# raulmur/ORB_SLAM2

Hardware: NVIDIA H100
Metric: stereo frames/sec (ORB extract L+R + ComputeStereoMatches, KITTI-shaped 1242x375 @2000 kpts) (higher is better)
Workload: dtype u8

## Files before the change

### orb_slam2_b200/csrc/borb_host.cu

```cuda
#include <cmath>
#include <cstdarg>
#include <cstdio>
#include <algorithm>
#include <cstdlib>
#include <cstring>

#include "borb_internal.h"

namespace borb {

static thread_local std::string tl_error;
void set_error(const char* fmt, ...) {
    char buf[512];
    va_list ap;
    va_start(ap, fmt);
    vsnprintf(buf, sizeof(buf), fmt, ap);
    va_end(ap);
    tl_error = buf;
}

bool allow_max_smem(const void* func) {
    static std::mutex mu;
    static std::vector<std::pair<const void*, int>> done;
    int dev = 0;
    if (cudaGetDevice(&dev) != cudaSuccess) return false;
    std::lock_guard<std::mutex> lk(mu);
    for (auto& d : done)
        if (d.first == func && d.second == dev) return true;
    cudaFuncAttributes fa;
    int optin = 0;
    cudaError_t e = cudaFuncGetAttributes(&fa, func);
    if (e == cudaSuccess) e = cudaDeviceGetAttribute(&optin, cudaDevAttrMaxSharedMemoryPerBlockOptin, dev);
    if (e == cudaSuccess) e = cudaFuncSetAttribute(func, cudaFuncAttributeMaxDynamicSharedMemorySize, optin - (int)fa.sharedSizeBytes);
    if (e != cudaSuccess) { set_error("raising the shared-memory limit failed: %s", cudaGetErrorString(e)); cudaGetLastError(); return false; }
    done.push_back({func, dev});
    return true;
}

namespace {

inline int cv_round_f(float v) { return (int)lrintf(v); }
inline int align_up(int v, int a) { return (v + a - 1) / a * a; }

void init_tables(borb_extractor* e) {
    const int L = e->cfg.n_levels;
    const double sf = (double)e->cfg.scale_factor;
    e->scale.assign(L, 1.f); e->sigma2.assign(L, 1.f); e->inv_scale.assign(L, 1.f); e->inv_sigma2.assign(L, 1.f);
    for (int i = 1; i < L; i++) {
        e->scale[i] = (float)((double)e->scale[i - 1] * sf);
        e->sigma2[i] = e->scale[i] * e->scale[i];
    }
    for (int i = 0; i < L; i++) { e->inv_scale[i] = 1.0f / e->scale[i]; e->inv_sigma2[i] = 1.0f / e->sigma2[i]; }
    e->per_level.assign(L, 0);
    const float factor = (float)(1.0 / sf);
    float want = (float)e->cfg.n_features * (1.f - factor) / (1.f - (float)std::pow((double)factor, (double)L));
    int sum = 0;
    for (int l = 0; l < L - 1; l++) {
        e->per_level[l] = cv_round_f(want);
        sum += e->per_level[l];
        want *= factor;
    }
    e->per_level[L - 1] = e->cfg.n_features - sum > 0 ? e->cfg.n_features - sum : 0;
    const int vmax = (int)std::floor(HALF_PATCH * std::sqrt(2.f) / 2 + 1);
    const int vmin = (int)std::ceil(HALF_PATCH * std::sqrt(2.f) / 2);
    for (int v = 0; v < 16; v++) e->umax[v] = 0;
    for (int v = 0; v <= vmax; ++v) e->umax[v] = (int)lrint(std::sqrt((double)HALF_PATCH * HALF_PATCH - (double)v * v));
    for (int v = HALF_PATCH, v0 = 0; v >= vmin; --v) {
        while (e->umax[v0] == e->umax[v0 + 1]) ++v0;
        e->umax[v] = v0;
        ++v0;
    }
}

void resize_table(int src, int dst, bool clamp_edges, int extra, std::vector<int16_t>& out) {
    const double inv = (double)dst / src, scale = 1. / inv;
    const size_t first = out.size();
    for (int d = 0; d < dst; d++) {
        float f = (float)((d + 0.5) * scale - 0.5);
        int s = (int)std::floor(f);
        f -= s;
        if (clamp_edges) {
            if (s < 0) { f = 0; s = 0; }
            if (s >= src - 1) { f = 0; s = src - 1; }
        }
        out.push_back((int16_t)s);
        out.push_back((int16_t)cv_round_f((1.f - f) * 2048.f));
        out.push_back((int16_t)cv_round_f(f * 2048.f));
        out.push_back(0);
    }
    for (int k = 0; k < extra; k++) {
        int r = 2 * dst - 2 - (dst + k);
        if (r < 0) r = 0;
        for (int j = 0; j < 4; j++) out.push_back(out[first + (size_t)r * 4 + j]);
    }
    if (((out.size() - first) / 4) & 1) for (int j = 0; j < 4; j++) out.push_back(0);
}

bool resize_window_table(const std::vector<int16_t>& tabs, size_t xtab_first, int n_entries, std::vector<int16_t>& out) {
    bool ok = true;
    for (int gq = 0; gq < n_entries; gq += 4) {
        int lo = 1 << 30, hi = 0;
        for (int i = 0; i < 4; i++) {
            const int ofs = tabs[xtab_first + (size_t)(gq + i) * 4];
            lo = std::min(lo, ofs); hi = std::max(hi, ofs);
        }
        const int base = lo & ~3;
        if (hi + 1 - base > 11) ok = false;
        for (int i = 0; i < 4; i++) {
            const int16_t* e = &tabs[xtab_first + (size_t)(gq + i) * 4];
            const int pos = e[0] - base;
            int s1 = 0, s2 = 0x10;
            if (pos <= 6) s1 = pos | ((pos + 1) << 4);
            else if (pos == 7) { s1 = 7; s2 = 0x40; }
            else { const int q = (pos - 8) + 4; s2 = q | ((q + 1) << 4); }
            out.push_back(e[1]);
            out.push_back(e[2]);
            out.push_back((int16_t)base);
            out.push_back((int16_t)((s1 | (s2 << 8)) & 0x7FFF));
        }
    }
    return ok;
}

const int8_t kPattern[1024] = {
#include "orb_pattern.inc"
};

borb_status build_geometry(borb_extractor* e, int w, int h, std::vector<int16_t>& tabs) {
    Geometry& g = e->geom;
    std::memset(&g, 0, sizeof(g));
    const int L = e->cfg.n_levels;
    g.nlevels = L; g.w = w; g.h = h;
    g.fast_mode = e->fast_mode;
    g.ini_th = e->cfg.ini_th_fast < 0 ? 0 : (e->cfg.ini_th_fast > 255 ? 255 : e->cfg.ini_th_fast);
    g.min_th = e->cfg.min_th_fast < 0 ? 0 : (e->cfg.min_th_fast > 255 ? 255 : e->cfg.min_th_fast);
    for (int i = 0; i < 16; i++) g.umax[i] = e->umax[i];
    unsigned pyr_off = 0, cand_off = 0;
    int blk = 0, sel_off = 0, btile = 0;
    tabs.clear();
    for (int l = 0; l < L; l++) {
        LevelGeom& v = g.lv[l];
        v.w = cv_round_f((float)w * e->inv_scale[l]);
        v.h = cv_round_f((float)h * e->inv_scale[l]);
        const float width = (float)(v.w - 2 * MIN_BORDER), height = (float)(v.h - 2 * MIN_BORDER);
        v.nCols = (int)(width / 30.f);
        v.nRows = (int)(height / 30.f);
        if (v.nCols < 1 || v.nRows < 1) {
            set_error("level %d is %dx%d: too small for the 30-px FAST cell grid (reference divides by zero)", l, v.w, v.h);
            return BORB_ERR_UNSUPPORTED;
        }
        v.wCell = (int)std::ceil(width / v.nCols);
        v.hCell = (int)std::ceil(height / v.nRows);
        v.pitch = align_up(v.w + 8, 128);
        v.pyr_off = pyr_off;
        pyr_off += (unsigned)v.pitch * v.h;
        v.cellsPerBlk = FAST_TILE_W / v.wCell > 0 ? FAST_TILE_W / v.wCell : 1;
        v.blkCols = (v.nCols + v.cellsPerBlk - 1) / v.cellsPerBlk;
        v.blkBase = blk;
        blk += v.blkCols * v.nRows;
        v.cand_off = cand_off;
        v.cand_cap = v.nCols * v.nRows * ((v.wCell + 1) / 2) * ((v.hCell + 1) / 2);
        cand_off += (unsigned)align_up(v.cand_cap, 32);
        v.quota = e->per_level[l];
        v.nIni = (int)std::round(width / height);
        if (v.nIni < 1) { set_error("level %d aspect ratio gives zero quadtree roots (reference divides by zero)", l); return BORB_ERR_UNSUPPORTED; }
        v.hX = width / v.nIni;
        v.node_cap = (v.quota > 4 * v.nIni ? v.quota : 4 * v.nIni) + 3;
        v.node_cap = align_up(v.node_cap + 1, 4);
        v.sel_off = sel_off;
        sel_off += v.node_cap;
        v.scale = e->scale[l];
        v.inv_scale = e->inv_scale[l];
        v.patch_size = (float)(int)(PATCH * e->scale[l]);
        g.blur_base[l] = btile;
        btile += ((v.w + BLUR_TILE_W - 1) / BLUR_TILE_W) * ((v.h + BLUR_TILE_H - 1) / BLUR_TILE_H);
        if (l > 0) {
            const int wpad = (v.w + 8 + 3) & ~3;
            v.xtab_off = (unsigned)(tabs.size() / 4);
            resize_table(g.lv[l - 1].w, v.w, true, wpad - v.w, tabs);
            v.ytab_off = (unsigned)(tabs.size() / 4);
            resize_table(g.lv[l - 1].h, v.h, false, 0, tabs);
            v.xwin_off = (unsigned)(tabs.size() / 4);
            std::vector<int16_t> win;
            v.x_windowed = resize_window_table(tabs, (size_t)v.xtab_off * 4, wpad, win) ? 1 : 0;
            tabs.insert(tabs.end(), win.begin(), win.end());
        }
        if (quadtree_smem_bytes(v.node_cap) > 200 * 1024) {
            set_error("per-level quota %d exceeds the quadtree kernel's shared-memory envelope", v.quota);
            return BORB_ERR_UNSUPPORTED;
        }
    }
    g.blur_base[L] = btile;
    g.blur_tiles = btile;
    g.fast_blocks = blk;
    g.pyr_image_stride = (unsigned)align_up((int)pyr_off, g.lv[0].pitch);
    g.cand_image_stride = cand_off;
    g.sel_image_stride = sel_off;
    if (sel_off >= 65536) { set_error("keypoint capacity %d exceeds 65535", sel_off); return BORB_ERR_UNSUPPORTED; }
    return BORB_OK;
}

void free_workspace(Workspace& ws) {
    cudaFree(ws.pyr); cudaFree(ws.blur); cudaFree(ws.cand); cudaFree(ws.cand_cnt); cudaFree(ws.pnode); cudaFree(ws.sel);
    cudaFree(ws.sel_cnt); cudaFree(ws.kps); cudaFree(ws.desc); cudaFree(ws.nkp); cudaFree(ws.u_right); cudaFree(ws.depth);
    cudaFree(ws.sad); cudaFree(ws.tabs); cudaFree(ws.brief_slots); cudaFree(ws.pair_idx); cudaFree(ws.st_bins); cudaFree(ws.st_recs); cudaFree(ws.stage);
    free(ws.fast_tmaps); cudaFree(ws.fast_tiles);
    ws = Workspace();
}

borb_status ensure(borb_extractor* e, int w, int h, int n_images) {
    if (w < 1 || h < 1 || w > BORB_MAX_DIM || h > BORB_MAX_DIM) { set_error("image size %dx%d outside [1,%d]", w, h, BORB_MAX_DIM); return BORB_ERR_UNSUPPORTED; }
    BORB_CUDA(cudaSetDevice(e->device));
    const bool same_shape = e->have_geom && e->geom.w == w && e->geom.h == h;
    if (same_shape && e->ws.max_images >= n_images) return BORB_OK;
    BORB_CUDA(cudaStreamSynchronize(e->stream));
    std::vector<int16_t> tabs;
    e->have_geom = false;
    e->last_n_images = 0;
    e->last_stereo_pairs = 0;
    borb_status st = build_geometry(e, w, h, tabs);
    if (st != BORB_OK) return st;
    size_t n = (size_t)(n_images > 2 ? n_images : 2);
    if (same_shape && (size_t)e->ws.max_images > n) n = (size_t)e->ws.max_images;
    free_workspace(e->ws);
    if (e->h_counts) { cudaFreeHost(e->h_counts); e->h_counts = nullptr; }
    e->pair_cache.clear();
    const Geometry& g = e->geom;
    Workspace& ws = e->ws;
    BORB_CUDA(cudaMalloc(&ws.pyr, n * g.pyr_image_stride + 256));
    BORB_CUDA(cudaMalloc(&ws.blur, n * g.pyr_image_stride + 256));
    BORB_CUDA(cudaMalloc(&ws.cand, n * g.cand_image_stride * sizeof(uint32_t)));
    BORB_CUDA(cudaMalloc(&ws.pnode, n * g.cand_image_stride * sizeof(int)));
    BORB_CUDA(cudaMalloc(&ws.cand_cnt, n * g.nlevels * sizeof(int)));
    BORB_CUDA(cudaMalloc(&ws.sel, n * g.sel_image_stride * sizeof(uint32_t)));
    BORB_CUDA(cudaMalloc(&ws.sel_cnt, n * g.nlevels * sizeof(int)));
    BORB_CUDA(cudaMalloc(&ws.kps, n * g.sel_image_stride * sizeof(borb_keypoint)));
    BORB_CUDA(cudaMalloc(&ws.desc, n * g.sel_image_stride * 32));
    BORB_CUDA(cudaMalloc(&ws.nkp, n * sizeof(int)));
    BORB_CUDA(cudaMalloc(&ws.u_right, n * g.sel_image_stride * sizeof(float)));
    BORB_CUDA(cudaMalloc(&ws.depth, n * g.sel_image_stride * sizeof(float)));
    BORB_CUDA(cudaMalloc(&ws.sad, n * g.sel_image_stride * sizeof(int)));
    BORB_CUDA(cudaMalloc(&ws.pair_idx, n * 2 * sizeof(int)));
    BORB_CUDA(cudaMalloc(&ws.st_bins, n * stereo_bins_bytes_per_pair()));
    BORB_CUDA(cudaMalloc(&ws.st_recs, n * (size_t)stereo_rec_stride(g) * stereo_rec_bytes()));
    BORB_CUDA(cudaMalloc(&ws.tabs, (tabs.size() + 4) * sizeof(int16_t)));
    BORB_CUDA(cudaMemcpy(ws.tabs, tabs.data(), tabs.size() * sizeof(int16_t), cudaMemcpyHostToDevice));
    const std::vector<uint32_t>& slots = brief_slot_table();
    BORB_CUDA(cudaMalloc(&ws.brief_slots, slots.size() * sizeof(uint32_t)));
    BORB_CUDA(cudaMemcpy(ws.brief_slots, slots.data(), slots.size() * sizeof(uint32_t), cudaMemcpyHostToDevice));
    BORB_CUDA(cudaMemset(ws.nkp, 0, n * sizeof(int)));
    BORB_CUDA(cudaMallocHost(&e->h_counts, n * 2 * sizeof(int)));
    ws.max_images = (int)n;
    ws.fast_tmaps = malloc(fast_tmaps_bytes());
    if ((st = build_fast_tmaps(g, ws, ws.fast_tmaps)) != BORB_OK) return st;
    if ((st = build_fast_tiles(g, ws)) != BORB_OK) return st;
    e->have_geom = true;
    return BORB_OK;
}

void drain_timing(borb_extractor* e);
void begin_step(borb_extractor* e) {
    if (!e->timing) return;
    if (e->ev.empty()) {
        e->ev.resize((size_t)borb_extractor::EV_RING * 9);
        for (auto& x : e->ev) cudaEventCreate(&x);
    }
    if (e->ev_pending >= borb_extractor::EV_RING) {
        cudaStreamSynchronize(e->stream);
        drain_timing(e);
    }
    e->ev_slot = (e->ev_slot + 1) % borb_extractor::EV_RING;
    e->ev_mask[e->ev_slot] = 0;
    e->ev_pending++;
}
void mark(borb_extractor* e, int i) {
    if (!e->timing || e->ev.empty()) return;
    cudaEventRecord(e->ev[(size_t)e->ev_slot * 9 + i], e->stream);
    e->ev_mask[e->ev_slot] |= 1u << i;
}
void drain_timing(borb_extractor* e) {
    const int R = borb_extractor::EV_RING;
    for (int k = e->ev_pending - 1; k >= 0; k--) {
        const int slot = ((e->ev_slot - k) % R + R) % R;
        const unsigned m = e->ev_mask[slot];
        for (int i = 0; i < 8; i++) {
            float ms = 0.f;
            if (m & (1u << i)) {
                int j = i + 1;
                while (j < 9 && !(m & (1u << j))) j++;
                if (j < 9 && cudaEventElapsedTime(&ms, e->ev[(size_t)slot * 9 + i], e->ev[(size_t)slot * 9 + j]) != cudaSuccess) { ms = 0.f; cudaGetLastError(); }
            }
            e->stage_ms[i] = ms;
            e->stage_sum_ms[i] += ms;
        }
        e->stage_steps++;
    }
    e->ev_pending = 0;
}

borb_status enqueue_extract(borb_extractor* e, int n) {
    const Geometry& g = e->geom;
    Workspace& ws = e->ws;
    cudaStream_t s = e->stream;
    BORB_CUDA(cudaMemsetAsync(ws.cand_cnt, 0, (size_t)n * g.nlevels * sizeof(int), s));
    mark(e, 1);
    e->launches += launch_pyramid(g, ws, n, s);
    mark(e, 2);
    e->launches += launch_fast(g, ws, n, s);
    mark(e, 3);
    e->launches += launch_quadtree(g, ws, n, s);
    mark(e, 4);
    e->launches += launch_blur(g, ws, n, s);
    mark(e, 5);
    e->launches += launch_describe(g, ws, n, s);
    mark(e, 6);
    BORB_CUDA(cudaGetLastError());
    e->last_n_images = n;
    e->last_stereo_pairs = 0;
    return BORB_OK;
}

borb_status rectified_size(borb_extractor* e, int w, int h, int* gw, int* gh) {
    if (!e->d_map[0][0]) return BORB_OK;
    if (w != e->map_src_w || h != e->map_src_h) {
        set_error("rectification maps were built for %dx%d raw frames, got %dx%d", e->map_src_w, e->map_src_h, w, h);
        return BORB_ERR_INVALID_ARG;
    }
    *gw = e->map_dst_w; *gh = e->map_dst_h;
    return BORB_OK;
}

borb_status upload_slots(borb_extractor* e, const uint8_t* const* slots, int n, int w, int h, int stride, bool stereo_pairs = false) {
    const Geometry& g = e->geom;
    const int ch = e->in_channels;
    if (stride < w * ch) { set_error("stride %d smaller than a row of %d %d-channel pixels", stride, w, ch); return BORB_ERR_INVALID_ARG; }
    const size_t img_bytes = (size_t)stride * h;
    bool contiguous = n > 1 || ch > 1 || e->d_map[0][0] != nullptr;
    for (int k = 0; k < n; k++) {
        if (!slots[k]) { set_error("image %d is NULL", k); return BORB_ERR_INVALID_ARG; }
        if (slots[k] != slots[0] + (size_t)k * img_bytes) contiguous = false;
    }
    auto need_stage = [&](size_t need) -> borb_status {
        if (e->ws.stage_bytes < need) {
            BORB_CUDA(cudaStreamSynchronize(e->stream));
            cudaFree(e->ws.stage);
            e->ws.stage = nullptr; e->ws.stage_bytes = 0;
            BORB_CUDA(cudaMalloc(&e->ws.stage, need));
            e->ws.stage_bytes = need;
        }
        return BORB_OK;
    };
    if (e->d_map[0][0]) {
        if (ch != 1) { set_error("rectification maps apply to CV_8UC1 frames"); return BORB_ERR_UNSUPPORTED; }
        const size_t src_img = contiguous ? img_bytes : (size_t)w * h;
        const int src_stride = contiguous ? stride : w;
        borb_status st = need_stage(src_img * n);
        if (st != BORB_OK) return st;
        if (contiguous) BORB_CUDA(cudaMemcpyAsync(e->ws.stage, slots[0], src_img * n, cudaMemcpyHostToDevice, e->stream));
        else
            for (int k = 0; k < n; k++)
                BORB_CUDA(cudaMemcpy2DAsync(e->ws.stage + (size_t)k * src_img, w, slots[k], stride, w, h, cudaMemcpyHostToDevice, e->stream));
        e->launches += launch_repack_remap(g, e->ws, e->ws.stage, src_stride, src_img, w, h, e->d_map[0][0], e->d_map[0][1],
                                           stereo_pairs ? e->d_map[1][0] : nullptr, stereo_pairs ? e->d_map[1][1] : nullptr, n, e->stream);
        return BORB_OK;
    }
    if (contiguous) {
        const size_t need = img_bytes * n;
        borb_status st = need_stage(need);
        if (st != BORB_OK) return st;
        BORB_CUDA(cudaMemcpyAsync(e->ws.stage, slots[0], need, cudaMemcpyHostToDevice, e->stream));
        if (ch == 1) e->launches += launch_repack(g, e->ws, e->ws.stage, stride, img_bytes, n, e->stream);
        else e->launches += launch_repack_color(g, e->ws, e->ws.stage, stride, img_bytes, ch, e->in_rgb, n, e->stream);
        return BORB_OK;
    }
    if (ch > 1) {
        const size_t row = (size_t)w * ch;
        borb_status st = need_stage(row * h * n);
        if (st != BORB_OK) return st;
        for (int k = 0; k < n; k++)
            BORB_CUDA(cudaMemcpy2DAsync(e->ws.stage + (size_t)k * row * h, row, slots[k], stride, row, h, cudaMemcpyHostToDevice, e->stream));
        e->launches += launch_repack_color(g, e->ws, e->ws.stage, (int)row, row * h, ch, e->in_rgb, n, e->stream);
        return BORB_OK;
    }
    for (int k = 0; k < n; k++) {
        uint8_t* dst = e->ws.pyr + (size_t)k * g.pyr_image_stride + g.lv[0].pyr_off;
        BORB_CUDA(cudaMemcpy2DAsync(dst, g.lv[0].pitch, slots[k], stride, w, h, cudaMemcpyHostToDevice, e->stream));
    }
    return BORB_OK;
}

borb_status upload_device(borb_extractor* e, const uint8_t* d_gray, int n, int w, int h, size_t pitch, size_t image_stride) {
    const Geometry& g = e->geom;
    cudaMemcpy3DParms p = {};
    p.srcPtr = make_cudaPitchedPtr((void*)d_gray, pitch, w, image_stride / pitch);
    p.dstPtr = make_cudaPitchedPtr(e->ws.pyr + g.lv[0].pyr_off, g.lv[0].pitch, w, g.pyr_image_stride / g.lv[0].pitch);
    if (image_stride % pitch == 0 && g.pyr_image_stride % g.lv[0].pitch == 0) {
        p.extent = make_cudaExtent(w, h, n);
        p.kind = cudaMemcpyDeviceToDevice;
        BORB_CUDA(cudaMemcpy3DAsync(&p, e->stream));
    } else {
        for (int i = 0; i < n; i++)
            BORB_CUDA(cudaMemcpy2DAsync(e->ws.pyr + (size_t)i * g.pyr_image_stride + g.lv[0].pyr_off, g.lv[0].pitch,
                                        d_gray + (size_t)i * image_stride, pitch, w, h, cudaMemcpyDeviceToDevice, e->stream));
    }
    return BORB_OK;
}

borb_status download_kps(borb_extractor* e, int first, int count, int step, borb_keypoint* kps, uint8_t* desc, int cap, int* n_out) {
    const Geometry& g = e->geom;
    const int m = cap < g.sel_image_stride ? cap : g.sel_image_stride;
    cudaStream_t s = e->stream;
    if (kps && m > 0)
        BORB_CUDA(cudaMemcpy2DAsync(kps, (size_t)cap * sizeof(borb_keypoint), e->ws.kps + (size_t)first * g.sel_image_stride,
                                    (size_t)step * g.sel_image_stride * sizeof(borb_keypoint), (size_t)m * sizeof(borb_keypoint),
                                    count, cudaMemcpyDeviceToHost, s));
    if (desc && m > 0)
        BORB_CUDA(cudaMemcpy2DAsync(desc, (size_t)cap * 32, e->ws.desc + (size_t)first * g.sel_image_stride * 32,
                                    (size_t)step * g.sel_image_stride * 32, (size_t)m * 32, count, cudaMemcpyDeviceToHost, s));
    if (n_out)
        BORB_CUDA(cudaMemcpy2DAsync(n_out, sizeof(int), e->ws.nkp + first, (size_t)step * sizeof(int), sizeof(int), count,
                                    cudaMemcpyDeviceToHost, s));
    return BORB_OK;
}

borb_status check_args(borb_extractor* e, int n, int w, int h) {
    if (!e) { set_error("null handle"); return BORB_ERR_INVALID_ARG; }
    if (n < 0) { set_error("negative image count"); return BORB_ERR_INVALID_ARG; }
    (void)w; (void)h;
    return BORB_OK;
}

borb_status enqueue_stereo(borb_extractor* eL, borb_extractor* eR, int n_pairs, const int* left_idx, const int* right_idx,
                           float bf, float b) {
    borb_extractor* e = eL;
    const Geometry& g = e->geom;
    std::vector<int> idx(2 * (size_t)n_pairs);
    for (int p = 0; p < n_pairs; p++) {
        idx[2 * p] = left_idx ? left_idx[p] : (eL == eR ? 2 * p : 0);
        idx[2 * p + 1] = right_idx ? right_idx[p] : (eL == eR ? 2 * p + 1 : 0);
        if (idx[2 * p] < 0 || idx[2 * p] >= eL->last_n_images || idx[2 * p + 1] < 0 || idx[2 * p + 1] >= eR->last_n_images) {
            set_error("stereo pair %d refers to an image outside the last batch", p);
            return BORB_ERR_STATE;
        }
    }
    if (n_pairs > e->ws.max_images) { set_error("too many pairs"); return BORB_ERR_INVALID_ARG; }
    if (idx != e->pair_cache) {
        BORB_CUDA(cudaStreamSynchronize(e->stream));
        std::memcpy(e->h_counts, idx.data(), idx.size() * sizeof(int));
        BORB_CUDA(cudaMemcpyAsync(e->ws.pair_idx, e->h_counts, idx.size() * sizeof(int), cudaMemcpyHostToDevice, e->stream));
        e->pair_cache = idx;
    }
    StereoView L{eL->ws.pyr, eL->ws.kps, eL->ws.desc, eL->ws.nkp, eL->geom.pyr_image_stride, eL->geom.sel_image_stride};
    StereoView R{eR->ws.pyr, eR->ws.kps, eR->ws.desc, eR->ws.nkp, eR->geom.pyr_image_stride, eR->geom.sel_image_stride};
    mark(e, 6);
    e->launches += launch_stereo(g, L, R, e->ws.pair_idx, n_pairs, bf, b, e->ws.u_right, e->ws.depth, e->ws.sad, g.sel_image_stride, e->ws.st_bins, e->ws.st_recs, e->stream);
    mark(e, 7);
    BORB_CUDA(cudaGetLastError());
    e->last_stereo_pairs = (eL == eR && !left_idx && !right_idx) ? n_pairs : 0;
    return BORB_OK;
}

borb_status download_stereo(borb_extractor* e, int n_pairs, float* u_right, float* depth, int cap) {
// ... 482 lines not shown
```

### orb_slam2_b200/csrc/borb_internal.h

```cpp
#pragma once
#include <cuda_runtime.h>
#include <stdint.h>

#include <mutex>
#include <string>
#include <vector>

#include "../../include/borb.h"

namespace borb {

constexpr int EDGE = 19;
constexpr int PATCH = 31;
constexpr int HALF_PATCH = 15;
constexpr int MIN_BORDER = 16;
constexpr int TH_HIGH = 100;
constexpr int TH_LOW = 50;
constexpr int BLUR_TILE_W = 120;
constexpr int BLUR_TILE_H = 64;
constexpr int FAST_TILE_W = 124;

__host__ __device__ inline uint32_t pack_xys(int x, int y, int s) { return (uint32_t)x | ((uint32_t)y << 12) | ((uint32_t)s << 24); }
__host__ __device__ inline int xys_x(uint32_t v) { return (int)(v & 0xFFFu); }
__host__ __device__ inline int xys_y(uint32_t v) { return (int)((v >> 12) & 0xFFFu); }
__host__ __device__ inline int xys_s(uint32_t v) { return (int)(v >> 24); }

struct LevelGeom {
    int w, h;
    int pitch;
    unsigned pyr_off;
    int nCols, nRows, wCell, hCell;
    int cellsPerBlk;
    int blkCols;
    int blkBase;
    unsigned cand_off;
    int cand_cap;
    int quota;
    int nIni;
    float hX;
    int node_cap;
    int sel_off;
    float scale;
    float inv_scale;
    float patch_size;
    unsigned xtab_off, ytab_off;
    unsigned xwin_off;
    int x_windowed;
};

struct Geometry {
    int nlevels;
    int w, h;
    int ini_th, min_th;
    int fast_mode;
    int fast_blocks;
    unsigned pyr_image_stride;
    unsigned cand_image_stride;
    int sel_image_stride;
    int blur_tiles;
    int blur_base[BORB_MAX_LEVELS + 1];
    int umax[16];
    LevelGeom lv[BORB_MAX_LEVELS];
};

struct Workspace {
    int max_images = 0;
    uint8_t* pyr = nullptr;
    uint8_t* blur = nullptr;
    uint32_t* cand = nullptr;
    int* cand_cnt = nullptr;
    int* pnode = nullptr;
    uint32_t* sel = nullptr;
    int* sel_cnt = nullptr;
    borb_keypoint* kps = nullptr;
    uint8_t* desc = nullptr;
    int* nkp = nullptr;
    float* u_right = nullptr;
    float* depth = nullptr;
    int* sad = nullptr;
    int16_t* tabs = nullptr;
    uint32_t* brief_slots = nullptr;
    int* pair_idx = nullptr;
    int* st_bins = nullptr;
    void* st_recs = nullptr;
    uint8_t* stage = nullptr;
    size_t stage_bytes = 0;
    void* fast_tmaps = nullptr;
    void* fast_tiles = nullptr;
    int fast_n_tiles = 0;
};

constexpr int BRIEF_BINS = 32;
const std::vector<uint32_t>& brief_slot_table();

void set_error(const char* fmt, ...);
bool allow_max_smem(const void* func);
#define BORB_CUDA(call)                                                                             \
    do {                                                                                            \
        cudaError_t _e = (call);                                                                    \
        if (_e != cudaSuccess) {                                                                    \
            borb::set_error("%s failed: %s (%s:%d)", #call, cudaGetErrorString(_e), __FILE__, __LINE__); \
            return (_e == cudaErrorNoDevice || _e == cudaErrorInsufficientDriver) ? BORB_ERR_NO_DEVICE : BORB_ERR_CUDA; \
        }                                                                                           \
    } while (0)

int launch_repack_remap(const Geometry& g, const Workspace& ws, const uint8_t* stage, int src_stride, size_t src_image_bytes, int src_w,
                        int src_h, const float* mx0, const float* my0, const float* mx1, const float* my1, int n_images, cudaStream_t s);
int launch_repack_color(const Geometry& g, const Workspace& ws, const uint8_t* stage, int src_stride, size_t src_image_bytes, int channels,
                        int rgb, int n_images, cudaStream_t s);
int launch_repack(const Geometry& g, const Workspace& ws, const uint8_t* stage, int src_stride, size_t src_image_bytes,
                  int n_images, cudaStream_t s);
int launch_pyramid(const Geometry& g, const Workspace& ws, int n_images, cudaStream_t s);
int launch_fast(const Geometry& g, const Workspace& ws, int n_images, cudaStream_t s);
int launch_quadtree(const Geometry& g, const Workspace& ws, int n_images, cudaStream_t s);
int launch_blur(const Geometry& g, const Workspace& ws, int n_images, cudaStream_t s);
int launch_describe(const Geometry& g, const Workspace& ws, int n_images, cudaStream_t s);

struct StereoView {
    const uint8_t* pyr;
    const borb_keypoint* kps;
    const uint8_t* desc;
    const int* nkp;
    unsigned pyr_image_stride;
    int kp_image_stride;
};
int launch_stereo(const Geometry& g, const StereoView& L, const StereoView& R, const int* d_pair_idx, int n_pairs,
                  float bf, float b, float* d_u_right, float* d_depth, int* d_sad, int out_stride, int* d_bins, void* d_recs,
                  cudaStream_t s);
int stereo_rec_stride(const Geometry& g);
size_t stereo_bins_bytes_per_pair();
size_t stereo_rec_bytes();
size_t quadtree_smem_bytes(int node_cap);
borb_status build_fast_tmaps(const Geometry& g, const Workspace& ws, void* out_tmaps);
borb_status build_fast_tiles(const Geometry& g, Workspace& ws);
size_t fast_tmaps_bytes();

}

struct borb_extractor {
    borb_extractor_cfg cfg;
    int device = 0;
    cudaStream_t stream = nullptr;
    std::vector<float> scale, inv_scale, sigma2, inv_sigma2;
    std::vector<int> per_level;
    int umax[16];
    bool have_geom = false;
    borb::Geometry geom;
    borb::Workspace ws;
    int last_n_images = 0;
    int last_stereo_pairs = 0;
    int in_channels = 1;
    int in_rgb = 1;
    float* d_map[2][2] = {{nullptr, nullptr}, {nullptr, nullptr}};
    int map_src_w = 0, map_src_h = 0, map_dst_w = 0, map_dst_h = 0;
    int fast_mode = 0;
    uint64_t launches = 0;
    static constexpr int EV_RING = 128;
    bool timing = false;
    std::vector<cudaEvent_t> ev;
    unsigned ev_mask[EV_RING] = {};
    int ev_slot = 0;
    int ev_pending = 0;
    float stage_ms[8] = {};
    double stage_sum_ms[8] = {};
    uint64_t stage_steps = 0;
    int* h_counts = nullptr;
    std::vector<int> pair_cache;
};
```

### orb_slam2_b200/csrc/k_fast.cu

```cuda
#include <cuda.h>

#include <cstring>

#include "borb_internal.h"

#include <algorithm>
#include <vector>

namespace borb {

namespace {

constexpr int TP = 160;
constexpr int TROWS = 66;
constexpr int QCAP = 60 * 128;

__device__ __forceinline__ uint32_t smem_u32(const void* p) { return (uint32_t)__cvta_generic_to_shared(p); }

template <int DX>
__device__ __forceinline__ uint32_t win(uint32_t W0, uint32_t W1, uint32_t W2) {
    if (DX == 0) return W1;
    if (DX > 0) return __byte_perm(W1, W2, DX | ((DX + 1) << 4) | ((DX + 2) << 8) | ((DX + 3) << 12));
    constexpr int K = 4 + DX;
    return __byte_perm(W0, W1, K | ((K + 1) << 4) | ((K + 2) << 8) | ((K + 3) << 12));
}

__device__ __forceinline__ uint32_t gt_flag(uint32_t q, uint32_t v, uint32_t K) {
    const uint32_t a = __vabsdiffu4(q, v);
    return (a + K) | a;
}

__device__ __forceinline__ uint32_t score_pair(const uint32_t (&d)[16], uint32_t v2) {
    uint32_t lo3[16], hi3[16];
#pragma unroll
    for (int k = 0; k < 16; k++) {
        lo3[k] = __vimin3_s16x2(d[k], d[(k + 1) & 15], d[(k + 2) & 15]);
        hi3[k] = __vimax3_s16x2(d[k], d[(k + 1) & 15], d[(k + 2) & 15]);
    }
    uint32_t lo9[16], hi9[16];
#pragma unroll
    for (int k = 0; k < 16; k++) {
        lo9[k] = __vimin3_s16x2(lo3[k], lo3[(k + 3) & 15], lo3[(k + 6) & 15]);
        hi9[k] = __vimax3_s16x2(hi3[k], hi3[(k + 3) & 15], hi3[(k + 6) & 15]);
    }
    uint32_t bb[5], dd[5];
#pragma unroll
    for (int k = 0; k < 5; k++) {
        bb[k] = __vimax3_s16x2(lo9[3 * k], lo9[3 * k + 1], lo9[3 * k + 2]);
        dd[k] = __vimin3_s16x2(hi9[3 * k], hi9[3 * k + 1], hi9[3 * k + 2]);
    }
    const uint32_t bright = __vimax3_s16x2(__vimax3_s16x2(bb[0], bb[1], bb[2]), __vimax3_s16x2(bb[3], bb[4], lo9[15]), bb[0]);
    const uint32_t darkm = __vimin3_s16x2(__vimin3_s16x2(dd[0], dd[1], dd[2]), __vimin3_s16x2(dd[3], dd[4], hi9[15]), dd[0]);
    return __viaddmax_s16x2_relu(__vmaxs2(__vsub2(bright, v2), __vsub2(v2, darkm)), 0xFFFFFFFFu, 0u);
}

__device__ __forceinline__ uint32_t score_pixels(const uint8_t* pa, const uint8_t* pb) {
    constexpr int RX[16] = {0, 1, 2, 3, 3, 3, 2, 1, 0, -1, -2, -3, -3, -3, -2, -1};
    constexpr int RY[16] = {3, 3, 2, 1, 0, -1, -2, -3, -3, -3, -2, -1, 0, 1, 2, 3};
    uint32_t d[16];
#pragma unroll
    for (int k = 0; k < 16; k++) {
        const int o = RY[k] * TP + RX[k];
        d[k] = (uint32_t)pa[o] | ((uint32_t)pb[o] << 16);
    }
    return score_pair(d, (uint32_t)pa[0] | ((uint32_t)pb[0] << 16));
}

}

struct TMaps { CUtensorMap m[BORB_MAX_LEVELS]; };

struct __align__(16) FastTile { int16_t l, ncell, x0, x1, y0, y1, wCell, hCell; };

__global__ void __launch_bounds__(256, 4) fast_kernel(const __grid_constant__ Geometry g, const __grid_constant__ TMaps tm,
                                                   const FastTile* __restrict__ tiles, uint32_t* __restrict__ cand, int* __restrict__ cand_cnt) {
    __shared__ __align__(128) uint8_t tile[TROWS * TP];
    __shared__ __align__(16) uint8_t score[60 * TP];
    __shared__ uint16_t queue[QCAP];
    __shared__ uint32_t wqueue[8 * 256];
    __shared__ __align__(8) unsigned long long bar;
    __shared__ int pn, qn, needB;
    __shared__ int cellHasIni[128 / 30 + 1];
    __shared__ uint8_t cellOf[128];

    const int img = blockIdx.y;
    const FastTile T = tiles[blockIdx.x];
    const int l = T.l, ncell = T.ncell, x0 = T.x0, x1 = T.x1, y0 = T.y0, y1 = T.y1;
    const int wCell = T.wCell, hCell = T.hCell;
    const LevelGeom& L = g.lv[l];
    const int tw = x1 - x0, th = y1 - y0;
    const int tid = threadIdx.x;
    const int lane = tid & 31, wrp = tid >> 5;

    const int xs = (x0 - 4) & ~15;
    const int off = x0 - xs;
    if (tid == 0) {
        asm volatile("mbarrier.init.shared::cta.b64 [%0], 1;" ::"r"(smem_u32(&bar)));
        asm volatile("fence.mbarrier_init.release.cluster;" ::: "memory");
        const uint32_t bytes = (uint32_t)TP * (uint32_t)(hCell + 6);
        asm volatile("mbarrier.arrive.expect_tx.shared::cta.b64 _, [%0], %1;" ::"r"(smem_u32(&bar)), "r"(bytes) : "memory");
        asm volatile(
            "cp.async.bulk.tensor.3d.shared::cluster.global.tile.mbarrier::complete_tx::bytes [%0], [%1, {%2, %3, %4}], [%5];"
            ::"r"(smem_u32(tile)), "l"(reinterpret_cast<uint64_t>(&tm.m[l])), "r"(xs), "r"(y0 - 3), "r"(img), "r"(smem_u32(&bar))
            : "memory");
    }
    if (tid < 128 / 30 + 1) cellHasIni[tid] = 0;
    if (tid < 128) cellOf[tid] = (uint8_t)(tid / wCell);
    if (tid == 0) { pn = 0; qn = 0; needB = 0; }
    __syncthreads();
    asm volatile(
        "{\n"
        ".reg .pred p;\n"
        "FAST_TMA_WAIT:\n"
        "mbarrier.try_wait.parity.shared::cta.b64 p, [%0], 0;\n"
        "@p bra FAST_TMA_DONE;\n"
        "bra FAST_TMA_WAIT;\n"
        "FAST_TMA_DONE:\n"
        "}\n" ::"r"(smem_u32(&bar))
        : "memory");
    if (g.fast_mode == 1) {
        if (reinterpret_cast<const uint32_t*>(tile)[tid] == 0x12345678u && cand_cnt[0] == -1) cand[0] = 1;
        return;
    }

    const uint32_t* T32 = reinterpret_cast<const uint32_t*>(tile);
    uint32_t* S32 = reinterpret_cast<uint32_t*>(score);
    const int wbase = off >> 2;
    const int wc = wbase + lane;
    uint32_t vmask = 0;
#pragma unroll
    for (int b = 0; b < 4; b++)
        if (4 * wc + b - off >= 0 && 4 * wc + b - off < tw) vmask |= 0x80u << (8 * b);

    auto collect = [&](int t, uint32_t m, bool zero) {
        const uint32_t K = (uint32_t)(127 - min(t, 127)) * 0x01010101u;
        asm volatile("" : "+r"(m));
        const bool reject = t <= 127;
        const int RG = (th + 7) >> 3;
        const int yBeg = wrp * RG, yEnd = min(th, yBeg + RG);
        uint32_t a0[7], a1[7], a2[7];
        int wcount = 0;
        if (yBeg < yEnd) {
#pragma unroll
            for (int j = 0; j < 6; j++) {
                const uint32_t* rp = T32 + (yBeg + j) * (TP / 4) + wc - 1;
                a0[j] = rp[0]; a1[j] = rp[1]; a2[j] = rp[2];
            }
        }
#pragma unroll
        for (int it = 0; it < 8; it++) {
            const int yy = yBeg + it;
            if (yy < yEnd) {
                {
                    const uint32_t* rp = T32 + (yy + 6) * (TP / 4) + wc - 1;
                    a0[(it + 6) % 7] = rp[0]; a1[(it + 6) % 7] = rp[1]; a2[(it + 6) % 7] = rp[2];
                }
#define ROW(dy) a0[(it + (dy) + 3) % 7], a1[(it + (dy) + 3) % 7], a2[(it + (dy) + 3) % 7]
                uint32_t f = m;
                if (reject && m) {
                    const uint32_t v = a1[(it + 3) % 7];
                    uint32_t acc = gt_flag(win<0>(ROW(3)), v, K) | gt_flag(win<0>(ROW(-3)), v, K);
                    acc &= gt_flag(win<2>(ROW(2)), v, K) | gt_flag(win<-2>(ROW(-2)), v, K);
                    acc &= gt_flag(win<3>(ROW(0)), v, K) | gt_flag(win<-3>(ROW(0)), v, K);
                    acc &= gt_flag(win<2>(ROW(-2)), v, K) | gt_flag(win<-2>(ROW(2)), v, K);
                    f = acc & m;
                }
#undef ROW
                const unsigned bal = __ballot_sync(0xFFFFFFFFu, f != 0);
                if (zero && m != 0) S32[yy * (TP / 4) + wc] = 0;
                if (f) wqueue[wrp * 256 + wcount + __popc(bal & ((1u << lane) - 1))] = f | (uint32_t)(yy << 8) | (uint32_t)wc;
                wcount += __popc(bal);
            }
        }
        __syncwarp();
        for (int i = 0; i < wcount; i += 32) {
            const uint32_t we = i + lane < wcount ? wqueue[wrp * 256 + i + lane] : 0u;
            const uint32_t fl = we & 0x80808080u;
            const int c = __popc(fl);
            int incl = c;
#pragma unroll
            for (int o2 = 1; o2 < 32; o2 <<= 1) {
                const int s = __shfl_up_sync(0xFFFFFFFFu, incl, o2);
                if (lane >= o2) incl += s;
            }
            int base = 0;
            if (lane == 31) base = atomicAdd(&pn, incl);
            base = __shfl_sync(0xFFFFFFFFu, base, 31) + incl - c;
            const int e = (int)((we >> 8) & 63) << 8 | (int)(4 * (we & 127));
#pragma unroll
            for (int b = 0; b < 4; b++)
                if (fl & (0x80u << (8 * b))) queue[base++] = (uint16_t)(e + b);
        }
    };

    auto score_queue = [&](int t) {
        const int np = pn;
        const int tc = max(t, 1);
        for (int rb = 0; rb < np; rb += 512) {
            const int e0 = rb + wrp * 64 + lane, e1 = e0 + 32;
            const bool va = e0 < np, vb = e1 < np;
            const int qa = va ? queue[e0] : off;
            const int qb = vb ? queue[e1] : qa;
            __syncthreads();
            if (rb + wrp * 64 < np) {
                const int ia = (qa >> 8) * TP + (qa & 255), ib = (qb >> 8) * TP + (qb & 255);
                const uint32_t s2 = score_pixels(tile + ia + 3 * TP, tile + ib + 3 * TP);
                const int sa = (int)(s2 & 0xFFFFu), sb = (int)(s2 >> 16);
                if (va) score[ia] = (uint8_t)sa;
                if (vb) score[ib] = (uint8_t)sb;
                const bool ca = va && sa >= tc, cb = vb && sb >= tc;
                if (__any_sync(0xFFFFFFFFu, ca || cb)) {
                    const int c = (int)ca + (int)cb;
                    int incl = c;
#pragma unroll
                    for (int o2 = 1; o2 < 32; o2 <<= 1) {
                        const int s = __shfl_up_sync(0xFFFFFFFFu, incl, o2);
                        if (lane >= o2) incl += s;
                    }
                    int base = 0;
                    if (lane == 31) base = atomicAdd(&qn, incl);
                    base = __shfl_sync(0xFFFFFFFFu, base, 31) + incl - c;
                    if (ca) queue[base++] = (uint16_t)qa;
                    if (cb) queue[base] = (uint16_t)qb;
                }
            }
        }
    };

    collect(g.ini_th, vmask, true);
    __syncthreads();
    if (g.fast_mode == 2) {
        if (pn == -1) cand[0] = 1;
        return;
    }
    score_queue(g.ini_th);
    __syncthreads();
    int nq = qn;
    if (g.fast_mode == 3) {
        if (nq == -1) cand[0] = 1;
        return;
    }

    uint32_t* out = cand + (size_t)img * g.cand_image_stride + L.cand_off;
    int* cnt = cand_cnt + img * g.nlevels + l;

    auto nms = [&](int n, bool mark) {
        for (int e = tid; e < n; e += 256) {
            const int q = queue[e];
            const int col = q & 255, yy = q >> 8;
            const int xx = col - off;
            const int s = score[yy * TP + col];
            const int c = cellOf[xx];
            const int cx0 = c * wCell, cx1 = min(cx0 + wCell, tw);
            bool ismax = true;
#pragma unroll
            for (int dy = -1; dy <= 1; dy++)
#pragma unroll
                for (int dx = -1; dx <= 1; dx++) {
                    if (dx == 0 && dy == 0) continue;
                    const int qx = xx + dx, qy = yy + dy;
                    if (qx < cx0 || qx >= cx1 || qy < 0 || qy >= th) continue;
                    if (!(s > (int)score[qy * TP + col + dx])) ismax = false;
                }
            if (ismax) {
                if (mark) cellHasIni[c] = 1;
            } else
                queue[e] = 0xFFFF;
        }
    };
    auto emit = [&](int n) {
        for (int eb = 0; eb < n; eb += 256) {
            const int e = eb + tid;
            int s = 0, xx = 0, yy = 0;
            if (e < n) {
                const int q = queue[e];
                if (q != 0xFFFF) {
                    const int col = q & 255;
                    yy = q >> 8; xx = col - off;
                    s = score[yy * TP + col];
                }
            }
            const unsigned m = __ballot_sync(0xFFFFFFFFu, s > 0);
            if (m) {
                int base = 0;
                if (lane == 0) base = atomicAdd(cnt, __popc(m));
                base = __shfl_sync(0xFFFFFFFFu, base, 0);
                if (s > 0) {
                    const int pos = base + __popc(m & ((1u << lane) - 1));
                    if (pos < L.cand_cap) out[pos] = pack_xys(x0 + xx, y0 + yy, s);
                }
            }
        }
    };

    nms(nq, true);
    __syncthreads();
    emit(nq);
    if (tid < ncell && tid * wCell < tw && !cellHasIni[tid] && g.min_th < g.ini_th) needB = 1;
    __syncthreads();
    if (!needB) return;

    {
        uint32_t need = 0;
#pragma unroll
        for (int b = 0; b < 4; b++) {
            const int xx = 4 * wc + b - off;
            if (xx >= 0 && xx < tw && !cellHasIni[cellOf[xx]]) need |= 0x80u << (8 * b);
        }
        if (tid == 0) { pn = 0; qn = 0; }
        __syncthreads();
        collect(g.min_th, need, false);
        __syncthreads();
        score_queue(g.min_th);
        __syncthreads();
        nq = qn;
        nms(nq, false);
        __syncthreads();
        emit(nq);
    }
}

typedef CUresult (*EncodeTiledFn)(CUtensorMap*, CUtensorMapDataType, cuuint32_t, void*, const cuuint64_t*, const cuuint64_t*,
                                  const cuuint32_t*, const cuuint32_t*, CUtensorMapInterleave, CUtensorMapSwizzle,
                                  CUtensorMapL2promotion, CUtensorMapFloatOOBfill);

borb_status build_fast_tmaps(const Geometry& g, const Workspace& ws, void* out_tmaps) {
    static EncodeTiledFn encode = nullptr;
    if (!encode) {
        void* fn = nullptr;
        cudaDriverEntryPointQueryResult qres;
        cudaError_t e = cudaGetDriverEntryPoint("cuTensorMapEncodeTiled", &fn, cudaEnableDefault, &qres);
        if (e != cudaSuccess || qres != cudaDriverEntryPointSuccess || !fn) {
            set_error("cuTensorMapEncodeTiled unavailable (%s)", cudaGetErrorString(e));
            return BORB_ERR_CUDA;
        }
        encode = (EncodeTiledFn)fn;
    }
    TMaps* tm = reinterpret_cast<TMaps*>(out_tmaps);
    std::memset(tm, 0, sizeof(TMaps));
    for (int l = 0; l < g.nlevels; l++) {
        const LevelGeom& L = g.lv[l];
        cuuint64_t dims[3] = {(cuuint64_t)L.w, (cuuint64_t)L.h, (cuuint64_t)ws.max_images};
        cuuint64_t strides[2] = {(cuuint64_t)L.pitch, (cuuint64_t)g.pyr_image_stride};
        cuuint32_t box[3] = {(cuuint32_t)TP, (cuuint32_t)(L.hCell + 6), 1};
        cuuint32_t estr[3] = {1, 1, 1};
        CUresult r = encode(&tm->m[l], CU_TENSOR_MAP_DATA_TYPE_UINT8, 3, ws.pyr + L.pyr_off, dims, strides, box, estr,
                            CU_TENSOR_MAP_INTERLEAVE_NONE, CU_TENSOR_MAP_SWIZZLE_NONE, CU_TENSOR_MAP_L2_PROMOTION_L2_128B,
                            CU_TENSOR_MAP_FLOAT_OOB_FILL_NONE);
        if (r != CUDA_SUCCESS) {
            set_error("cuTensorMapEncodeTiled failed for level %d (CUresult %d)", l, (int)r);
            return BORB_ERR_CUDA;
        }
    }
    return BORB_OK;
}

size_t fast_tmaps_bytes() { return sizeof(TMaps); }

borb_status build_fast_tiles(const Geometry& g, Workspace& ws) {
    std::vector<FastTile> t;
    for (int l = 0; l < g.nlevels; l++) {
        const LevelGeom& L = g.lv[l];
        for (int cellRow = 0; cellRow < L.nRows; cellRow++)
            for (int blkCol = 0; blkCol < L.blkCols; blkCol++) {
                const int cell0 = blkCol * L.cellsPerBlk;
                const int ncell = std::min(L.cellsPerBlk, L.nCols - cell0);
                const int x0 = EDGE + cell0 * L.wCell, x1 = std::min(x0 + ncell * L.wCell, L.w - EDGE);
                const int y0 = EDGE + cellRow * L.hCell, y1 = std::min(y0 + L.hCell, L.h - EDGE);
                if (x0 >= x1 || y0 >= y1) continue;
                FastTile f;
                f.l = (int16_t)l; f.ncell = (int16_t)ncell; f.x0 = (int16_t)x0; f.x1 = (int16_t)x1; f.y0 = (int16_t)y0; f.y1 = (int16_t)y1;
                f.wCell = (int16_t)L.wCell; f.hCell = (int16_t)L.hCell;
                t.push_back(f);
            }
    }
    cudaFree(ws.fast_tiles); ws.fast_tiles = nullptr;
    ws.fast_n_tiles = (int)t.size();
    if (t.empty()) return BORB_OK;
    BORB_CUDA(cudaMalloc(&ws.fast_tiles, t.size() * sizeof(FastTile)));
    BORB_CUDA(cudaMemcpy(ws.fast_tiles, t.data(), t.size() * sizeof(FastTile), cudaMemcpyHostToDevice));
    return BORB_OK;
}

int launch_fast(const Geometry& g, const Workspace& ws, int n_images, cudaStream_t s) {
    if (ws.fast_n_tiles == 0) return 0;
    dim3 grid(ws.fast_n_tiles, n_images);
    fast_kernel<<<grid, 256, 0, s>>>(g, *reinterpret_cast<const TMaps*>(ws.fast_tmaps), reinterpret_cast<const FastTile*>(ws.fast_tiles), ws.cand, ws.cand_cnt);
    return 1;
}

}
```

Measured before the change: 35030.

## Band multiple FAST cell rows per CTA to cut halo reloads and block count

The FAST kernel now processes a vertical band of up to 64 pixel rows, which can span several cell rows, in each CTA instead of a single cell row. The TMA box, tile list, per-cell NMS bounds, cellHasIni bookkeeping and the fallback mask are extended to track cell rows within the band, and shared memory moves to a dynamic allocation. This aims to reduce the number of CTAs and the redundant 6-row halo loads. The costs are more shared memory per CTA, which may lower occupancy, and extra per-row mask selection in the inner loop.

```diff
diff --git a/orb_slam2_b200/csrc/borb_host.cu b/orb_slam2_b200/csrc/borb_host.cu
--- a/orb_slam2_b200/csrc/borb_host.cu
+++ b/orb_slam2_b200/csrc/borb_host.cu
@@ -155,9 +155,10 @@
         v.pyr_off = pyr_off;
         pyr_off += (unsigned)v.pitch * v.h;
         v.cellsPerBlk = FAST_TILE_W / v.wCell > 0 ? FAST_TILE_W / v.wCell : 1;
+        v.rowsPerBlk = fast_rows_per_blk(v.nRows, v.hCell);
         v.blkCols = (v.nCols + v.cellsPerBlk - 1) / v.cellsPerBlk;
         v.blkBase = blk;
-        blk += v.blkCols * v.nRows;
+        blk += v.blkCols * ((v.nRows + v.rowsPerBlk - 1) / v.rowsPerBlk);
         v.cand_off = cand_off;
         v.cand_cap = v.nCols * v.nRows * ((v.wCell + 1) / 2) * ((v.hCell + 1) / 2);
         cand_off += (unsigned)align_up(v.cand_cap, 32);
diff --git a/orb_slam2_b200/csrc/borb_internal.h b/orb_slam2_b200/csrc/borb_internal.h
--- a/orb_slam2_b200/csrc/borb_internal.h
+++ b/orb_slam2_b200/csrc/borb_internal.h
@@ -19,6 +19,13 @@
 constexpr int BLUR_TILE_W = 120;
 constexpr int BLUR_TILE_H = 64;
 constexpr int FAST_TILE_W = 124;
+constexpr int FAST_H_BAND = 64;
+
+__host__ __device__ inline int fast_rows_per_blk(int nRows, int hCell) {
+    const int r = FAST_H_BAND / hCell;
+    return r < 1 ? 1 : (r > nRows ? nRows : r);
+}
+__host__ __device__ inline int fast_box_rows(int rowsPerBlk, int hCell) { return rowsPerBlk * hCell + 6; }
 
 __host__ __device__ inline uint32_t pack_xys(int x, int y, int s) { return (uint32_t)x | ((uint32_t)y << 12) | ((uint32_t)s << 24); }
 __host__ __device__ inline int xys_x(uint32_t v) { return (int)(v & 0xFFFu); }
@@ -31,6 +38,7 @@
     unsigned pyr_off;
     int nCols, nRows, wCell, hCell;
     int cellsPerBlk;
+    int rowsPerBlk;
     int blkCols;
     int blkBase;
     unsigned cand_off;
diff --git a/orb_slam2_b200/csrc/k_fast.cu b/orb_slam2_b200/csrc/k_fast.cu
--- a/orb_slam2_b200/csrc/k_fast.cu
+++ b/orb_slam2_b200/csrc/k_fast.cu
@@ -5,6 +5,7 @@
 #include "borb_internal.h"
 
 #include <algorithm>
+#include <type_traits>
 #include <vector>
 
 namespace borb {
@@ -12,8 +13,17 @@
 namespace {
 
 constexpr int TP = 160;
-constexpr int TROWS = 66;
-constexpr int QCAP = 60 * 128;
+constexpr int HB = FAST_H_BAND;
+static_assert(HB >= 60 && HB <= 127, "a one-row band (hCell <= 59) must fit; collect packs the row into 7 bits");
+constexpr int TROWS = HB + 6;
+constexpr int QCAP = HB * 128;
+constexpr int RG_MAX = (HB + 7) / 8;
+constexpr int WSEG = RG_MAX * 32;
+constexpr int RMAX = HB / 30;
+constexpr int NCX = 128 / 30 + 1;
+constexpr int SM_SCORE = TROWS * TP, SM_QUEUE = SM_SCORE + HB * TP, SM_WQUEUE = SM_QUEUE + QCAP * 2;
+constexpr int FAST_SMEM = SM_WQUEUE + 8 * WSEG * 4;
+static_assert(SM_SCORE % 16 == 0 && SM_WQUEUE % 4 == 0, "shared-memory carve-up alignment");
 
 __device__ __forceinline__ uint32_t smem_u32(const void* p) { return (uint32_t)__cvta_generic_to_shared(p); }
 
@@ -70,18 +80,21 @@
 
 struct TMaps { CUtensorMap m[BORB_MAX_LEVELS]; };
 
-struct __align__(16) FastTile { int16_t l, ncell, x0, x1, y0, y1, wCell, hCell; };
+struct __align__(16) FastTile { int8_t l, ncell, rowsPerBlk, pad; int16_t x0, x1, y0, y1, wCell, hCell; };
+static_assert(sizeof(FastTile) == 16, "one 16-byte load per CTA");
 
 __global__ void __launch_bounds__(256, 4) fast_kernel(const __grid_constant__ Geometry g, const __grid_constant__ TMaps tm,
                                                    const FastTile* __restrict__ tiles, uint32_t* __restrict__ cand, int* __restrict__ cand_cnt) {
-    __shared__ __align__(128) uint8_t tile[TROWS * TP];
-    __shared__ __align__(16) uint8_t score[60 * TP];
-    __shared__ uint16_t queue[QCAP];
-    __shared__ uint32_t wqueue[8 * 256];
+    extern __shared__ __align__(128) uint8_t smem[];
+    uint8_t* tile = smem;
+    uint8_t* score = smem + SM_SCORE;
+    uint16_t* queue = reinterpret_cast<uint16_t*>(smem + SM_QUEUE);
+    uint32_t* wqueue = reinterpret_cast<uint32_t*>(smem + SM_WQUEUE);
     __shared__ __align__(8) unsigned long long bar;
     __shared__ int pn, qn, needB;
-    __shared__ int cellHasIni[128 / 30 + 1];
+    __shared__ int cellHasIni[RMAX * NCX];
     __shared__ uint8_t cellOf[128];
+    __shared__ uint8_t rowOf[HB];
 
     const int img = blockIdx.y;
     const FastTile T = tiles[blockIdx.x];
@@ -97,15 +110,16 @@
     if (tid == 0) {
         asm volatile("mbarrier.init.shared::cta.b64 [%0], 1;" ::"r"(smem_u32(&bar)));
         asm volatile("fence.mbarrier_init.release.cluster;" ::: "memory");
-        const uint32_t bytes = (uint32_t)TP * (uint32_t)(hCell + 6);
+        const uint32_t bytes = (uint32_t)TP * (uint32_t)fast_box_rows(T.rowsPerBlk, hCell);
         asm volatile("mbarrier.arrive.expect_tx.shared::cta.b64 _, [%0], %1;" ::"r"(smem_u32(&bar)), "r"(bytes) : "memory");
         asm volatile(
             "cp.async.bulk.tensor.3d.shared::cluster.global.tile.mbarrier::complete_tx::bytes [%0], [%1, {%2, %3, %4}], [%5];"
             ::"r"(smem_u32(tile)), "l"(reinterpret_cast<uint64_t>(&tm.m[l])), "r"(xs), "r"(y0 - 3), "r"(img), "r"(smem_u32(&bar))
             : "memory");
     }
-    if (tid < 128 / 30 + 1) cellHasIni[tid] = 0;
+    if (tid < RMAX * NCX) cellHasIni[tid] = 0;
     if (tid < 128) cellOf[tid] = (uint8_t)(tid / wCell);
+    if (tid < HB) rowOf[tid] = (uint8_t)(tid / hCell);
     if (tid == 0) { pn = 0; qn = 0; needB = 0; }
     __syncthreads();
     asm volatile(
@@ -132,9 +146,15 @@
     for (int b = 0; b < 4; b++)
         if (4 * wc + b - off >= 0 && 4 * wc + b - off < tw) vmask |= 0x80u << (8 * b);
 
-    auto collect = [&](int t, uint32_t m, bool zero) {
+    auto collect = [&](int t, const uint32_t (&mr)[RMAX], bool zero, auto banded) {
+        constexpr bool BANDED = decltype(banded)::value;
         const uint32_t K = (uint32_t)(127 - min(t, 127)) * 0x01010101u;
-        asm volatile("" : "+r"(m));
+        uint32_t mm[RMAX];
+#pragma unroll
+        for (int r = 0; r < (BANDED ? RMAX : 1); r++) {
+            mm[r] = mr[r];
+            asm volatile("" : "+r"(mm[r]));
+        }
         const bool reject = t <= 127;
         const int RG = (th + 7) >> 3;
         const int yBeg = wrp * RG, yEnd = min(th, yBeg + RG);
@@ -147,13 +167,20 @@
                 a0[j] = rp[0]; a1[j] = rp[1]; a2[j] = rp[2];
             }
         }
-#pragma unroll
-        for (int it = 0; it < 8; it++) {
-            const int yy = yBeg + it;
+        for (int it0 = 0; it0 < RG; it0 += 7)
+#pragma unroll
+        for (int it = 0; it < 7; it++) {
+            const int yy = yBeg + it0 + it;
             if (yy < yEnd) {
                 {
                     const uint32_t* rp = T32 + (yy + 6) * (TP / 4) + wc - 1;
                     a0[(it + 6) % 7] = rp[0]; a1[(it + 6) % 7] = rp[1]; a2[(it + 6) % 7] = rp[2];
+                }
+                uint32_t m = mm[0];
+                if constexpr (BANDED) {
+#pragma unroll
+                    for (int r = 1; r < RMAX; r++)
+                        if (yy >= r * hCell) m = mm[r];
                 }
 #define ROW(dy) a0[(it + (dy) + 3) % 7], a1[(it + (dy) + 3) % 7], a2[(it + (dy) + 3) % 7]
                 uint32_t f = m;
@@ -168,13 +195,13 @@
 #undef ROW
                 const unsigned bal = __ballot_sync(0xFFFFFFFFu, f != 0);
                 if (zero && m != 0) S32[yy * (TP / 4) + wc] = 0;
-                if (f) wqueue[wrp * 256 + wcount + __popc(bal & ((1u << lane) - 1))] = f | (uint32_t)(yy << 8) | (uint32_t)wc;
+                if (f) wqueue[wrp * WSEG + wcount + __popc(bal & ((1u << lane) - 1))] = f | (uint32_t)(yy << 8) | (uint32_t)wc;
                 wcount += __popc(bal);
             }
         }
         __syncwarp();
         for (int i = 0; i < wcount; i += 32) {
-            const uint32_t we = i + lane < wcount ? wqueue[wrp * 256 + i + lane] : 0u;
+            const uint32_t we = i + lane < wcount ? wqueue[wrp * WSEG + i + lane] : 0u;
             const uint32_t fl = we & 0x80808080u;
             const int c = __popc(fl);
             int incl = c;
@@ -186,7 +213,7 @@
             int base = 0;
             if (lane == 31) base = atomicAdd(&pn, incl);
             base = __shfl_sync(0xFFFFFFFFu, base, 31) + incl - c;
-            const int e = (int)((we >> 8) & 63) << 8 | (int)(4 * (we & 127));
+            const int e = (int)((we >> 8) & 127) << 8 | (int)(4 * (we & 127));
 #pragma unroll
             for (int b = 0; b < 4; b++)
                 if (fl & (0x80u << (8 * b))) queue[base++] = (uint16_t)(e + b);
@@ -227,7 +254,10 @@
         }
     };
 
-    collect(g.ini_th, vmask, true);
+    {
+        const uint32_t mA[RMAX] = {vmask};
+        collect(g.ini_th, mA, true, std::false_type());
+    }
     __syncthreads();
     if (g.fast_mode == 2) {
         if (pn == -1) cand[0] = 1;
@@ -250,8 +280,9 @@
             const int col = q & 255, yy = q >> 8;
             const int xx = col - off;
             const int s = score[yy * TP + col];
-            const int c = cellOf[xx];
+            const int c = cellOf[xx], r = rowOf[yy];
             const int cx0 = c * wCell, cx1 = min(cx0 + wCell, tw);
+            const int cy0 = r * hCell, cy1 = min(cy0 + hCell, th);
             bool ismax = true;
 #pragma unroll
             for (int dy = -1; dy <= 1; dy++)
@@ -259,11 +290,11 @@
                 for (int dx = -1; dx <= 1; dx++) {
                     if (dx == 0 && dy == 0) continue;
                     const int qx = xx + dx, qy = yy + dy;
-                    if (qx < cx0 || qx >= cx1 || qy < 0 || qy >= th) continue;
+                    if (qx < cx0 || qx >= cx1 || qy < cy0 || qy >= cy1) continue;
                     if (!(s > (int)score[qy * TP + col + dx])) ismax = false;
                 }
             if (ismax) {
-                if (mark) cellHasIni[c] = 1;
+                if (mark) cellHasIni[r * NCX + c] = 1;
             } else
                 queue[e] = 0xFFFF;
         }
@@ -296,20 +327,27 @@
     nms(nq, true);
     __syncthreads();
     emit(nq);
-    if (tid < ncell && tid * wCell < tw && !cellHasIni[tid] && g.min_th < g.ini_th) needB = 1;
+    if (tid < RMAX * NCX) {
+        const int r = tid / NCX, c = tid - r * NCX;
+        if (r * hCell < th && c < ncell && c * wCell < tw && !cellHasIni[tid] && g.min_th < g.ini_th) needB = 1;
+    }
     __syncthreads();
     if (!needB) return;
 
     {
-        uint32_t need = 0;
-#pragma unroll
-        for (int b = 0; b < 4; b++) {
-            const int xx = 4 * wc + b - off;
-            if (xx >= 0 && xx < tw && !cellHasIni[cellOf[xx]]) need |= 0x80u << (8 * b);
+        uint32_t need[RMAX];
+#pragma unroll
+        for (int r = 0; r < RMAX; r++) {
+            need[r] = 0;
+#pragma unroll
+            for (int b = 0; b < 4; b++) {
+                const int xx = 4 * wc + b - off;
+                if (xx >= 0 && xx < tw && !cellHasIni[r * NCX + cellOf[xx]]) need[r] |= 0x80u << (8 * b);
+            }
         }
         if (tid == 0) { pn = 0; qn = 0; }
         __syncthreads();
-        collect(g.min_th, need, false);
+        collect(g.min_th, need, false, std::true_type());
         __syncthreads();
         score_queue(g.min_th);
         __syncthreads();
@@ -342,7 +380,7 @@
         const LevelGeom& L = g.lv[l];
         cuuint64_t dims[3] = {(cuuint64_t)L.w, (cuuint64_t)L.h, (cuuint64_t)ws.max_images};
         cuuint64_t strides[2] = {(cuuint64_t)L.pitch, (cuuint64_t)g.pyr_image_stride};
-        cuuint32_t box[3] = {(cuuint32_t)TP, (cuuint32_t)(L.hCell + 6), 1};
+        cuuint32_t box[3] = {(cuuint32_t)TP, (cuuint32_t)fast_box_rows(L.rowsPerBlk, L.hCell), 1};
         cuuint32_t estr[3] = {1, 1, 1};
         CUresult r = encode(&tm->m[l], CU_TENSOR_MAP_DATA_TYPE_UINT8, 3, ws.pyr + L.pyr_off, dims, strides, box, estr,
                             CU_TENSOR_MAP_INTERLEAVE_NONE, CU_TENSOR_MAP_SWIZZLE_NONE, CU_TENSOR_MAP_L2_PROMOTION_L2_128B,
@@ -361,15 +399,17 @@
     std::vector<FastTile> t;
     for (int l = 0; l < g.nlevels; l++) {
         const LevelGeom& L = g.lv[l];
-        for (int cellRow = 0; cellRow < L.nRows; cellRow++)
+        for (int cellRow = 0; cellRow < L.nRows; cellRow += L.rowsPerBlk)
             for (int blkCol = 0; blkCol < L.blkCols; blkCol++) {
                 const int cell0 = blkCol * L.cellsPerBlk;
                 const int ncell = std::min(L.cellsPerBlk, L.nCols - cell0);
+                const int nrow = std::min(L.rowsPerBlk, L.nRows - cellRow);
                 const int x0 = EDGE + cell0 * L.wCell, x1 = std::min(x0 + ncell * L.wCell, L.w - EDGE);
-                const int y0 = EDGE + cellRow * L.hCell, y1 = std::min(y0 + L.hCell, L.h - EDGE);
+                const int y0 = EDGE + cellRow * L.hCell, y1 = std::min(y0 + nrow * L.hCell, L.h - EDGE);
                 if (x0 >= x1 || y0 >= y1) continue;
                 FastTile f;
-                f.l = (int16_t)l; f.ncell = (int16_t)ncell; f.x0 = (int16_t)x0; f.x1 = (int16_t)x1; f.y0 = (int16_t)y0; f.y1 = (int16_t)y1;
+                f.l = (int8_t)l; f.ncell = (int8_t)ncell; f.rowsPerBlk = (int8_t)L.rowsPerBlk; f.pad = 0;
+                f.x0 = (int16_t)x0; f.x1 = (int16_t)x1; f.y0 = (int16_t)y0; f.y1 = (int16_t)y1;
                 f.wCell = (int16_t)L.wCell; f.hCell = (int16_t)L.hCell;
                 t.push_back(f);
             }
@@ -384,8 +424,9 @@
 
 int launch_fast(const Geometry& g, const Workspace& ws, int n_images, cudaStream_t s) {
     if (ws.fast_n_tiles == 0) return 0;
+    allow_max_smem((const void*)fast_kernel);
     dim3 grid(ws.fast_n_tiles, n_images);
-    fast_kernel<<<grid, 256, 0, s>>>(g, *reinterpret_cast<const TMaps*>(ws.fast_tmaps), reinterpret_cast<const FastTile*>(ws.fast_tiles), ws.cand, ws.cand_cnt);
+    fast_kernel<<<grid, 256, FAST_SMEM, s>>>(g, *reinterpret_cast<const TMaps*>(ws.fast_tmaps), reinterpret_cast<const FastTile*>(ws.fast_tiles), ws.cand, ws.cand_cnt);
     return 1;
 }
 
```

New measurement: 36990, median of 6. 1.06x the previous value.
